# AdamQLMeng/PPNet

Hardware: AMD Instinct MI355X
Metric: edage_pp_map_path_instances_per_sec (higher is better)
Workload: dtype f64

## Files before the change

### include/ppnet_hip.h

```cpp
#ifndef PPNET_HIP_H
#define PPNET_HIP_H

#include <stdint.h>

#ifdef __cplusplus
extern "C" {
#endif

#define PPN_OK             0
#define PPN_E_INVALID     -1
#define PPN_E_HIP         -2
#define PPN_E_UNSUPPORTED -3

#define PPN_SEGS            10
#define PPN_POLY             5
#define PPN_PATH_POINTS   1000
#define PPN_BOUNDARY_POINTS 1100
#define PPN_DRAWS_PER_SEG 1002
#define PPN_DRAWS_PER_PATH (1 + PPN_SEGS * PPN_DRAWS_PER_SEG)
#define PPN_MAX_HULL        64
#define PPN_MAX_ISLES       16
#define PPN_MAX_POCKET      64
#define PPN_POCKET_TRY_CAP 256
#define PPN_PLACE_TRY_CAP 4096
// ... 285 lines not shown
                      void* stream);
#define PPN_AUG_FLIP            1u
#define PPN_AUG_BRIGHTNESS      2u
#define PPN_AUG_CONTRAST        4u
#define PPN_AUG_CONTRAST_LAST   8u
#define PPN_AUG_SATURATION     16u
#define PPN_AUG_HUE            32u
#define PPN_AUG_PARAM_WORDS     8
int ppn_augment_params(uint64_t seed, uint64_t first_instance, int B, double flip_ratio, double brightness_delta, double contrast_lo,
                       double contrast_hi, double saturation_lo, double saturation_hi, int hue_delta,
                       uint32_t* params , void* stream);
int ppn_augment_codes(const uint8_t* grid , const uint8_t* label_in ,
                      const uint32_t* params , void* img_out ,
                      uint8_t* label_out , int B, int H, int W, int Ho, int Wo,
                      const float* mean3, const float* std3, int seg_pad_val, int dtype , void* stream);
int ppn_augment_rgb(const uint8_t* rgb , const uint8_t* label_in ,
                    const uint32_t* params , void* img_out ,
                    uint8_t* label_out , int B, int H, int W, int Ho, int Wo,
                    const float* mean3, const float* std3, int seg_pad_val, int dtype , void* stream);
int ppn_seg_labels_2class(const void* logits, uint8_t* labels, int32_t B, int32_t h, int32_t w, int32_t Ho, int32_t Wo,
                          int32_t dtype, void* stream);
int ppn_bias_act_nhwc(void* x, const void* bias, int64_t n, int32_t C, float negative_slope, int32_t dtype, void* stream);

int ppn_conv3x3_c1_nhwc(const void* x, const float* w, const float* bias, void* y, int32_t B, int32_t H, int32_t W,
                        int32_t Cout, float negative_slope, int32_t dtype, void* stream);
int ppn_conv3x3_to1_nhwc(const void* x, const float* w, float bias, void* y, int32_t B, int32_t H, int32_t W, int32_t Cin,
                         int32_t dtype, void* stream);

int ppn_conv3x3_mfma_bf16(const void* x, const void* w, const float* bias, void* y, int32_t B, int32_t H, int32_t W, int32_t Cin,
                          int32_t Cout, int32_t stride, int32_t relu, void* stream);
int32_t ppn_conv3x3_relu_classify2_slots(int32_t Cout);
int ppn_conv3x3_relu_classify2_bf16(const void* x, const void* w, const float* bias, const float* w2, float* logits, float* partial, int32_t B,
                                    int32_t H, int32_t W, int32_t Cin, int32_t Cout, void* stream);
int ppn_gennet_conv_s2_bf16(const void* x, const void* w, const float* bias, void* y, int32_t B, int32_t H, int32_t W, float negative_slope,
                            int32_t transposed, void* stream);
int ppn_gennet_dec_final_bf16(const void* x, const void* w, const float* bias, float negative_slope, const float* w_final, float bias_final, void* y,
                              int32_t B, int32_t H, int32_t W, void* stream);
int ppn_gennet_first_enc_bf16(const void* x1, const void* w1, const float* b1, const void* wk2, const float* bias2, void* y, int32_t B, int32_t H, int32_t W,
                              float slope1, float slope2, void* stream);
#define PPN_GENNET_BLOCK_PARAMS 7224
int ppn_gennet_trunk_bf16(const void* x, void* y, const float* params, int32_t B, int32_t N, int32_t n_blocks, void* stream);
int ppn_assemble_paths(const double* wp, const int32_t* wp_n, const uint8_t* ok, const double* init, const double* end, double rate, int32_t n,
                       int32_t max_wp, double* full, int32_t* counts, void* stream);
int ppn_plan_collision(const double* waypoints, const int32_t* counts, const void* obstacles, int32_t obstacles_f64, const int32_t* n_obstacles,
                       int32_t B, int32_t M, int32_t S, float clearance, float bound, uint8_t* collision, void* stream);
int ppn_heatmap_u8(const void* y, uint8_t* out, int32_t B, int32_t n, int32_t dtype, void* stream);
int ppn_tokenizer_conv1_codes_bf16(const uint8_t* grid, const void* lut, void* out, int32_t B, int32_t H, int32_t W, void* stream);
int ppn_tokenizer_codes_bf16(const uint8_t* grid, const void* lut, const void* w2p, const float* vec, void* tokens, int32_t B, int32_t H, int32_t W,
                             float eps, void* stream);
int ppn_nat128_ln_qkv_bf16(const void* s, const float* offset, const void* ln_w, const void* ln_b, const void* w, const void* bias, void* qkv,
                           int64_t tokens, float eps, void* stream);
int ppn_nat128_ln_mlp_bf16(void* s, const float* offset, const void* ln_w, const void* ln_b, const void* w1, const void* b1, const void* w2,
                           int64_t tokens, float eps, void* stream);
int ppn_nat128_ln_mlp_add_bf16(void* s, const float* offset, const void* ln_w, const void* ln_b, const void* w1, const void* b1, const void* w2,
                               const float* final_add, int64_t tokens, float eps, void* stream);
int ppn_nat128_proj_add_bf16(void* s, const void* a, const void* w, int64_t tokens, void* stream);

int ppn_gemm_bf16(const void* a, const void* w, const float* bias, void* c, int64_t M, int32_t N, int32_t K, int32_t epilogue,
                  int32_t persistent_blocks, void* stream);

int32_t ppn_nat_gemm_partials(int32_t C);

int ppn_nat_gemm_bf16(const void* a, const void* w, const float* bias, const float* colsum, const float* stats_in, int32_t partials_in,
                      float* stats_out, void* c, int64_t M, int32_t N, int32_t K, int32_t mode, float eps, void* stream);

int32_t ppn_nat_mlp_supported(int64_t M, int32_t C, int32_t HID);
// ... 17 lines not shown
```

### ppnet_amd/_lib.py

```python
import ctypes as C
import os

_HERE = os.path.dirname(os.path.abspath(__file__))
LIB_PATH = os.environ.get("PPNET_HIP_LIB") or os.path.join(_HERE, "libppnet_hip.so")

PPN_OK = 0
PPN_E_UNSUPPORTED = -3
SEGS = 10
PATH_POINTS = 1000
BOUNDARY_POINTS = 1100
DRAWS_PER_SEG = 1002
DRAWS_PER_PATH = 1 + SEGS * DRAWS_PER_SEG
MAX_HULL = 64
MAX_ISLES = 16
MAX_POCKET = 64
POCKET_TRY_CAP = 256
PLACE_TRY_CAP = 4096
MAX_WAYPOINTS = 2048
GRID_OBST, GRID_FREE, GRID_MARK = 0, 255, 128
FLAG_POCKET_CAP, FLAG_PLACE_CAP, FLAG_EMPTY_ISLE, FLAG_HULL_CAP, FLAG_ISLE_CAP, FLAG_POCKET_FULL = 1, 2, 4, 8, 16, 32
FLAG_CORRIDOR_PASS = 64
FLAG_POCKET_DRAWS = 128

_p = C.c_void_p
# ... 9 lines not shown

class MapsStruct(C.Structure):
    _fields_ = [(n, _p) for n in (
        "grid", "angle", "translation", "attempts", "segpoint", "pathpoint", "accept", "obstacles",
        "n_obstacles", "flags", "records")]


class TtaAug(C.Structure):
    _fields_ = [("logit", _p), ("h", C.c_int32), ("w", C.c_int32), ("hm", C.c_int32), ("wm", C.c_int32), ("flip", C.c_int32)]


ABI_VERSION = 111

EXPORTS = ("ppn_version", "ppn_error_string", "ppn_last_hip_error", "ppn_polyfit_table", "ppn_edage_paths",
           "ppn_edage_paths_ex", "ppn_edage_paths_ex2", "ppn_edage_maps", "ppn_edage_maps_place", "ppn_edage_maps_raster",
           "ppn_label_masks", "ppn_boundary_check", "ppn_boundary_check_ex",
           "ppn_obstacle_filter", "ppn_paint_markers", "ppn_disc_raster", "ppn_collision_segments", "ppn_collision_segments_bound",
           "ppn_extract_paths", "ppn_resize_bilinear_u8", "ppn_philox_doubles", "ppn_na2d_fwd", "ppn_na2d_fwd_padded", "ppn_na2d_fwd_vpad", "ppn_swin_wmsa_fwd", "ppn_swin_wmsa_bwd", "ppn_swin_wmsa_bwd_workspace", "ppn_mhsa_fwd", "ppn_mhsa_bwd", "ppn_mhsa_bwd_workspace", "ppn_na2d_bwd", "ppn_na2d_bwd_workspace", "ppn_na2d_bwd_vpad", "ppn_na2d_bwd_vpad_workspace", "ppn_residual_layernorm", "ppn_residual_layernorm_padded", "ppn_layernorm_offset", "ppn_upsample2x_nhwc", "ppn_resize_concat4_nhwc", "ppn_resize_concat_nhwc", "ppn_adaptive_pools_nhwc", "ppn_upsample2x_add_nhwc", "ppn_upsample2x_nhwc_bias", "ppn_upsample2x_concat_nhwc", "ppn_bias_act_nhwc", "ppn_seg_labels_2class", "ppn_grid_to_image", "ppn_conv3x3_c1_nhwc", "ppn_conv3x3_to1_nhwc",
           "ppn_conv3x3_mfma_bf16", "ppn_conv3x3_relu_classify2_bf16", "ppn_conv3x3_relu_classify2_slots", "ppn_gemm_bf16", "ppn_nat_gemm_bf16", "ppn_nat_gemm_partials", "ppn_row_stats_bf16", "ppn_nat_mlp_supported", "ppn_nat_mlp_pack_bf16", "ppn_nat_mlp_bf16", "ppn_gennet_conv_s2_bf16", "ppn_gennet_trunk_bf16",
           "ppn_assemble_paths", "ppn_plan_collision", "ppn_gennet_first_enc_bf16", "ppn_gennet_dec_final_bf16", "ppn_heatmap_u8", "ppn_tokenizer_conv1_codes_bf16", "ppn_tokenizer_codes_bf16", "ppn_nat128_ln_qkv_bf16", "ppn_nat128_ln_mlp_bf16", "ppn_nat128_ln_mlp_add_bf16", "ppn_nat128_proj_add_bf16",
           "ppn_resize_ce_workspace", "ppn_resize_ce_fwd", "ppn_resize_ce_bwd", "ppn_seg_eval",
           "ppn_augment_params", "ppn_augment_codes", "ppn_augment_rgb",
           "ppn_ohem_ce_workspace", "ppn_ohem_ce_fwd", "ppn_ohem_ce_bwd",
           "ppn_resize_dice_workspace", "ppn_resize_dice_fwd", "ppn_resize_dice_bwd",
           "ppn_upsample2x_nhwc_bwd", "ppn_upsample2x_concat_nhwc_bwd", "ppn_resize_concat_nhwc_bwd",
           "ppn_residual_layernorm_train_fwd", "ppn_residual_layernorm_bwd_workspace", "ppn_residual_layernorm_bwd",
           "ppn_patch_merge_ln_fwd", "ppn_patch_merge_ln_bwd_workspace", "ppn_patch_merge_ln_bwd", "ppn_patch_merge_ln_rows",
           "ppn_patch_merge_ln_max_blocks", "ppn_seg_tta",
           "ppn_gennet_stem_train_workspace", "ppn_gennet_stem_train_fwd", "ppn_gennet_stem_train_bwd", "ppn_gennet_stem_train_tile",
           "ppn_gennet_stem_train_max_blocks",
           "ppn_gennet_tail_train_workspace", "ppn_gennet_tail_train_fwd", "ppn_gennet_tail_train_bwd", "ppn_gennet_tail_train_tile",
           "ppn_gennet_tail_train_max_blocks",
           "ppn_gennet_s2_tile", "ppn_gennet_s2_max_blocks", "ppn_gennet_s2_wgrad_workspace", "ppn_gennet_s2_down", "ppn_gennet_s2_up",
           "ppn_gennet_s2_wgrad")


def _load():
    if not os.path.exists(LIB_PATH):
        raise ImportError(
            f"{LIB_PATH} is missing: the HIP extension is the only implementation of this package "
            f"(no CPU fallback). Build it with `python -c 'import __graft_entry__ as g; g.build()'` "
            f"or `make -C ppnet_amd/csrc`.")
    lib = C.CDLL(LIB_PATH)
    lib.ppn_version.restype = C.c_int
    if lib.ppn_version() != ABI_VERSION:
        raise ImportError(
            f"{LIB_PATH} reports ABI version {lib.ppn_version()}, these bindings are written against {ABI_VERSION} "
            f"(include/ppnet_hip.h: PPN_ABI_VERSION): argument lists differ, rebuild with `make -C ppnet_amd/csrc`.")
    lib.ppn_error_string.restype = C.c_char_p
    lib.ppn_error_string.argtypes = [C.c_int]
    lib.ppn_last_hip_error.restype = C.c_int
    lib.ppn_polyfit_table.argtypes = [_p]
    lib.ppn_edage_paths.argtypes = [C.c_int32, C.c_uint64, C.c_int32, C.c_double, C.c_double, C.c_uint64,
                                    _p, _p, C.c_int32, C.POINTER(PathsStruct), _p]
    lib.ppn_edage_paths_ex.argtypes = [C.c_int32, C.c_uint64, C.c_int32, C.c_double, C.c_double, C.c_uint64,
                                       _p, _p, C.c_int32, _p, C.POINTER(PathsStruct), _p]
    lib.ppn_edage_paths_ex2.argtypes = [C.c_int32, C.c_uint64, C.c_int32, C.c_double, C.c_double, C.c_uint64,
                                        _p, _p, C.c_int32, _p, _p, C.POINTER(PathsStruct), _p]
    lib.ppn_boundary_check_ex.argtypes = [_p, C.c_int32, _p, _p, C.c_int32, C.c_int32, _p, _p, _p]
    lib.ppn_obstacle_filter.argtypes = [_p, _p, C.c_int32, C.c_int32, C.c_int32, C.c_double, C.c_double, C.c_double,
                                        _p, _p, _p, _p]
    lib.ppn_paint_markers.argtypes = [_p, C.c_int32, C.c_int32, _p, _p, _p]
    lib.ppn_edage_maps.argtypes = [C.POINTER(PathsStruct), C.c_int32, C.c_int32, C.c_uint64, C.c_int32,
                                   C.c_double, C.c_double, C.c_int32, C.c_double, C.c_uint64, _p, _p,
                                   C.POINTER(MapsStruct), _p]
    lib.ppn_edage_maps_place.argtypes = lib.ppn_edage_maps.argtypes
    lib.ppn_edage_maps_raster.argtypes = [C.POINTER(PathsStruct), C.c_int32, C.c_int32, C.c_int32, C.c_int32,
# ... 48 lines not shown
    lib.ppn_patch_merge_ln_fwd.argtypes = [_p] * 5 + [C.c_int] * 4 + [C.c_float, C.c_int, _p]
    lib.ppn_patch_merge_ln_bwd_workspace.argtypes = [C.c_int] * 4
    lib.ppn_patch_merge_ln_bwd_workspace.restype = C.c_int64
    lib.ppn_patch_merge_ln_bwd.argtypes = [_p] * 8 + [C.c_int] * 5 + [_p]
    lib.ppn_patch_merge_ln_rows.argtypes = [C.c_int]
    lib.ppn_patch_merge_ln_max_blocks.argtypes = []
    lib.ppn_gennet_stem_train_workspace.argtypes = [C.c_int] * 4
    lib.ppn_gennet_stem_train_workspace.restype = C.c_int64
    lib.ppn_gennet_stem_train_fwd.argtypes = [_p] * 9 + [C.c_int] * 4 + [C.c_float, C.c_float, C.c_int, _p]
    lib.ppn_gennet_stem_train_bwd.argtypes = [_p] * 12 + [C.c_int] * 4 + [C.c_float, C.c_int, _p]
    lib.ppn_gennet_stem_train_tile.argtypes = []
    lib.ppn_gennet_stem_train_max_blocks.argtypes = []
    lib.ppn_gennet_tail_train_workspace.argtypes = [C.c_int] * 4
    lib.ppn_gennet_tail_train_workspace.restype = C.c_int64
    lib.ppn_gennet_tail_train_fwd.argtypes = [_p] * 8 + [C.c_int] * 4 + [C.c_float, C.c_float, C.c_int, _p]
    lib.ppn_gennet_tail_train_bwd.argtypes = [_p] * 12 + [C.c_int] * 4 + [C.c_float, C.c_int, _p]
    lib.ppn_gennet_tail_train_tile.argtypes = []
    lib.ppn_gennet_tail_train_max_blocks.argtypes = []
    lib.ppn_gennet_s2_tile.argtypes = []
    lib.ppn_gennet_s2_max_blocks.argtypes = []
    lib.ppn_gennet_s2_wgrad_workspace.argtypes = [C.c_int] * 3
    lib.ppn_gennet_s2_wgrad_workspace.restype = C.c_int64
    lib.ppn_gennet_s2_down.argtypes = [_p] * 4 + [C.c_int] * 5 + [_p]
    lib.ppn_gennet_s2_up.argtypes = [_p] * 4 + [C.c_int] * 5 + [_p]
    lib.ppn_gennet_s2_wgrad.argtypes = [_p] * 6 + [C.c_int] * 5 + [_p]
    lib.ppn_grid_to_image.argtypes = [_p, _p, C.c_int64, C.POINTER(C.c_float), C.POINTER(C.c_float), C.c_int32, _p]
    lib.ppn_seg_labels_2class.argtypes = [_p, _p, C.c_int32, C.c_int32, C.c_int32, C.c_int32, C.c_int32, C.c_int32, _p]
    lib.ppn_bias_act_nhwc.argtypes = [_p, _p, C.c_int64, C.c_int32, C.c_float, C.c_int32, _p]
    lib.ppn_conv3x3_c1_nhwc.argtypes = [_p, _p, _p, _p, C.c_int32, C.c_int32, C.c_int32, C.c_int32, C.c_float, C.c_int32, _p]
    lib.ppn_conv3x3_to1_nhwc.argtypes = [_p, _p, C.c_float, _p, C.c_int32, C.c_int32, C.c_int32, C.c_int32, C.c_int32, _p]
    lib.ppn_conv3x3_mfma_bf16.argtypes = [_p, _p, _p, _p, C.c_int32, C.c_int32, C.c_int32, C.c_int32, C.c_int32, C.c_int32, C.c_int32, _p]
    lib.ppn_conv3x3_relu_classify2_bf16.argtypes = [_p, _p, _p, _p, _p, _p, C.c_int32, C.c_int32, C.c_int32, C.c_int32, C.c_int32, _p]
    lib.ppn_conv3x3_relu_classify2_slots.argtypes = [C.c_int32]
    lib.ppn_gennet_conv_s2_bf16.argtypes = [_p, _p, _p, _p, C.c_int32, C.c_int32, C.c_int32, C.c_float, C.c_int32, _p]
    lib.ppn_gennet_trunk_bf16.argtypes = [_p, _p, _p, C.c_int32, C.c_int32, C.c_int32, _p]
    lib.ppn_assemble_paths.argtypes = [_p, _p, _p, _p, _p, C.c_double, C.c_int32, C.c_int32, _p, _p, _p]
    lib.ppn_plan_collision.argtypes = [_p, _p, _p, C.c_int32, _p, C.c_int32, C.c_int32, C.c_int32, C.c_float, C.c_float, _p, _p]
    lib.ppn_gennet_first_enc_bf16.argtypes = [_p, _p, _p, _p, _p, _p, C.c_int32, C.c_int32, C.c_int32, C.c_float, C.c_float, _p]
    lib.ppn_gennet_dec_final_bf16.argtypes = [_p, _p, _p, C.c_float, _p, C.c_float, _p, C.c_int32, C.c_int32, C.c_int32, _p]
    lib.ppn_heatmap_u8.argtypes = [_p, _p, C.c_int32, C.c_int32, C.c_int32, _p]
    lib.ppn_tokenizer_conv1_codes_bf16.argtypes = [_p, _p, _p, C.c_int32, C.c_int32, C.c_int32, _p]
    lib.ppn_tokenizer_codes_bf16.argtypes = [_p, _p, _p, _p, _p, C.c_int32, C.c_int32, C.c_int32, C.c_float, _p]
    lib.ppn_nat128_ln_qkv_bf16.argtypes = [_p, _p, _p, _p, _p, _p, _p, C.c_int64, C.c_float, _p]
    lib.ppn_nat128_ln_mlp_bf16.argtypes = [_p, _p, _p, _p, _p, _p, _p, C.c_int64, C.c_float, _p]
    lib.ppn_nat128_ln_mlp_add_bf16.argtypes = [_p, _p, _p, _p, _p, _p, _p, _p, C.c_int64, C.c_float, _p]
    lib.ppn_nat128_proj_add_bf16.argtypes = [_p, _p, _p, C.c_int64, _p]
    lib.ppn_gemm_bf16.argtypes = [_p, _p, _p, _p, C.c_int64, C.c_int32, C.c_int32, C.c_int32, C.c_int32, _p]
    lib.ppn_nat_gemm_bf16.argtypes = [_p, _p, _p, _p, _p, C.c_int32, _p, _p, C.c_int64, C.c_int32, C.c_int32, C.c_int32, C.c_float, _p]
    lib.ppn_row_stats_bf16.argtypes = [_p, C.c_int64, C.c_int32, _p, _p]
    lib.ppn_nat_gemm_partials.argtypes = [C.c_int32]
    lib.ppn_nat_mlp_supported.argtypes = [C.c_int64, C.c_int32, C.c_int32]
    lib.ppn_nat_mlp_pack_bf16.argtypes = [_p, _p, _p, C.c_int32, C.c_int32, _p]
    lib.ppn_nat_mlp_bf16.argtypes = [_p, _p, _p, _p, _p, C.c_int64, C.c_int32, C.c_int32, C.c_float, _p]
    lib.ppn_resize_ce_workspace.argtypes = [C.c_int] * 3
    lib.ppn_resize_ce_workspace.restype = C.c_int64
    lib.ppn_resize_ce_fwd.argtypes = [_p, _p, _p, _p, _p, _p, C.c_int64] + [C.c_int] * 9 + [_p]
    lib.ppn_resize_ce_bwd.argtypes = [_p, _p, _p, _p, _p] + [C.c_int] * 9 + [_p]
    lib.ppn_seg_eval.argtypes = [_p, _p, _p, _p] + [C.c_int] * 9 + [_p]
    lib.ppn_seg_tta.argtypes = [C.POINTER(TtaAug), C.c_int, _p, _p] + [C.c_int] * 5 + [_p]
    lib.ppn_ohem_ce_workspace.argtypes = [C.c_int] * 3
    lib.ppn_ohem_ce_workspace.restype = C.c_int64
    lib.ppn_ohem_ce_fwd.argtypes = [_p] * 10 + [C.c_int64] + [C.c_int] * 8 + [C.c_float] + [C.c_int] * 3 + [_p]
    lib.ppn_ohem_ce_bwd.argtypes = [_p] * 8 + [C.c_int] * 10 + [_p]
    lib.ppn_resize_dice_workspace.argtypes = [C.c_int] * 4
    lib.ppn_resize_dice_workspace.restype = C.c_int64
    lib.ppn_resize_dice_fwd.argtypes = [_p] * 8 + [C.c_int] * 7 + [C.c_float] + [C.c_int] * 2 + [_p]
# ... 32 lines not shown
```

### ppnet_amd/csrc/capi.hip

```cpp
#include <hip/hip_runtime.h>
#include <math.h>
#include <mutex>
#include <stdlib.h>
#include <string.h>
#include <vector>

#include <cstdlib>
#include "ppn_kernels.h"

namespace {

thread_local int g_last_hip = 0;

inline int hip_fail(hipError_t e) {
    g_last_hip = (int)e;
    return PPN_E_HIP;
}
#define PPN_HIP(call) do { hipError_t e_ = (call); if (e_ != hipSuccess) return hip_fail(e_); } while (0)

inline bool bad_R(int R) { return R < 32 || R > 512 || (R % 32) != 0; }

void build_polyfit_table(double* out) {
    const int N = PPN_PATH_POINTS, M = 5;
    std::vector<long double> q((size_t)M * N);
// ... 1086 lines not shown
                         void* stream) {
    if (!x || !w || !y || B <= 0 || H <= 0 || W <= 0 || Cin <= 0 || Cin > 32 || (Cin % 8) != 0 || (dtype != 0 && dtype != 1))
        return PPN_E_INVALID;
    const int e = ppn::conv3x3_to1_launch(x, w, bias, y, B, H, W, Cin, dtype, (hipStream_t)stream);
    if (e != 0) return hip_fail((hipError_t)e);
    return PPN_OK;
}

int ppn_conv3x3_mfma_bf16(const void* x, const void* w, const float* bias, void* y, int32_t B, int32_t H, int32_t W, int32_t Cin,
                          int32_t Cout, int32_t stride, int32_t relu, void* stream) {
    if (!x || !w || !bias || !y || B <= 0 || H <= 0 || W <= 0 || Cin <= 0 || (Cin % 64) != 0 || Cout <= 0 || (Cout % 8) != 0 ||
        (stride != 1 && stride != 2))
        return PPN_E_INVALID;
    if ((long long)B * H * W * Cin * 2 >= (1LL << 32) || (long long)Cout * 9 * Cin * 2 >= (1LL << 32) || (long long)B * H * W >= (1LL << 31))
        return PPN_E_UNSUPPORTED;
    const int e = ppn::conv3x3_mfma_launch(x, w, bias, y, B, H, W, Cin, Cout, stride, relu, nullptr, nullptr, nullptr, (hipStream_t)stream);
    if (e != 0) return hip_fail((hipError_t)e);
    return PPN_OK;
}

int32_t ppn_conv3x3_relu_classify2_slots(int32_t Cout) { return Cout > 0 ? (Cout > 256 ? (Cout + 255) / 256 : 0) : -1; }

int ppn_conv3x3_relu_classify2_bf16(const void* x, const void* w, const float* bias, const float* w2, float* logits, float* partial, int32_t B,
                                    int32_t H, int32_t W, int32_t Cin, int32_t Cout, void* stream) {
    if (!x || !w || !bias || !w2 || !logits || (!partial && Cout > 256) || B <= 0 || H <= 0 || W <= 0 || Cin <= 0 || (Cin % 64) != 0 || Cout <= 0 || (Cout % 8) != 0)
        return PPN_E_INVALID;
    if ((long long)B * H * W * Cin * 2 >= (1LL << 32) || (long long)Cout * 9 * Cin * 2 >= (1LL << 32) || (long long)B * H * W >= (1LL << 31))
        return PPN_E_UNSUPPORTED;
    const int e = ppn::conv3x3_mfma_launch(x, w, bias, nullptr, B, H, W, Cin, Cout, 1, 1, w2, logits, partial, (hipStream_t)stream);
    if (e != 0) return hip_fail((hipError_t)e);
    return PPN_OK;
}

int ppn_gennet_conv_s2_bf16(const void* x, const void* w, const float* bias, void* y, int32_t B, int32_t H, int32_t W, float negative_slope,
                            int32_t transposed, void* stream) {
    if (!x || !w || !bias || !y || B <= 0 || H <= 0 || W <= 0 || (!transposed && ((H | W) & 1))) return PPN_E_INVALID;
    if ((long long)B * H * W * 4 >= (1LL << 31)) return PPN_E_UNSUPPORTED;
    const int e = transposed ? ppn::gennet_dec_conv_launch(x, w, bias, y, B, H, W, negative_slope, (hipStream_t)stream)
                             : ppn::gennet_enc_conv_launch(x, w, bias, y, B, H, W, negative_slope, (hipStream_t)stream);
    if (e != 0) return hip_fail((hipError_t)e);
    return PPN_OK;
}

int ppn_gennet_first_enc_bf16(const void* x1, const void* w1, const float* b1, const void* wk2, const float* bias2, void* y, int32_t B, int32_t H, int32_t W,
                              float slope1, float slope2, void* stream) {
    if (!x1 || !w1 || !b1 || !wk2 || !bias2 || !y || B <= 0 || H <= 0 || W <= 0 || ((H | W) & 1)) return PPN_E_INVALID;
    const int e = ppn::gennet_first_enc_launch(x1, w1, b1, wk2, bias2, y, B, H, W, slope1, slope2, (hipStream_t)stream);
    if (e != 0) return hip_fail((hipError_t)e);
    return PPN_OK;
}

int ppn_gennet_dec_final_bf16(const void* x, const void* w, const float* bias, float negative_slope, const float* w_final, float bias_final, void* y,
                              int32_t B, int32_t H, int32_t W, void* stream) {
    if (!x || !w || !bias || !w_final || !y || B <= 0 || H <= 0 || W <= 0) return PPN_E_INVALID;
    if ((long long)B * H * W * 4 * 24 >= (1LL << 32)) return PPN_E_UNSUPPORTED;
    const int e = ppn::gennet_dec_final_launch(x, w, bias, negative_slope, w_final, bias_final, y, B, H, W, (hipStream_t)stream);
    if (e != 0) return hip_fail((hipError_t)e);
    return PPN_OK;
}

int ppn_gennet_trunk_bf16(const void* x, void* y, const float* params, int32_t B, int32_t N, int32_t n_blocks, void* stream) {
    if (!x || !y || !params || B <= 0 || N <= 0 || N > 1024 || (N % 8) != 0 || n_blocks <= 0) return PPN_E_INVALID;
    const int e = ppn::gennet_trunk_launch(x, y, params, B, N, n_blocks, (hipStream_t)stream);
    if (e != 0) return hip_fail((hipError_t)e);
    return PPN_OK;
}
// ... 163 lines not shown
```

### ppnet_amd/csrc/ppn_kernels.h

```cpp
#pragma once
#include <hip/hip_runtime.h>
#include <stdint.h>
#include <atomic>
#include "../../include/ppnet_hip.h"

#ifndef PPN_PATHS_THREADS
#define PPN_PATHS_THREADS 256
#endif

namespace ppn {

constexpr int PPN_MAX_DEVICES = 64;
inline int current_device() {
    int d = 0;
    return (hipGetDevice(&d) == hipSuccess && d >= 0 && d < PPN_MAX_DEVICES) ? d : -1;
}
struct DeviceOnce { std::atomic<int> done[PPN_MAX_DEVICES]; };
struct DeviceBuffer { std::atomic<void*> p[PPN_MAX_DEVICES]; };
inline int dynamic_lds_once(DeviceOnce& o, const void* fn, int bytes) {
    const int d = current_device();
    if (d < 0) return (int)hipErrorInvalidDevice;
    if (o.done[d].load(std::memory_order_acquire)) return 0;
    const hipError_t e = hipFuncSetAttribute(fn, hipFuncAttributeMaxDynamicSharedMemorySize, bytes);
    if (e != hipSuccess) return (int)e;
// ... 116 lines not shown
int gennet_tail_tile();
int gennet_tail_max_blocks();
long long gennet_tail_train_workspace_bytes(long long n, int C);
int gennet_tail_train_fwd_launch(const void* y, const float* gamma, const float* beta, const float* wf, const float* bf, void* out, float* stats,
                                 void* workspace, int B, int H, int W, int C, float eps, float slope, int dtype, hipStream_t stream);
int gennet_tail_train_bwd_launch(const void* dout, const void* y, const float* gamma, const float* beta, const float* wf, const float* stats,
                                 void* workspace, void* dy, float* dgamma, float* dbeta, float* dwf, float* dbf, int B, int H, int W, int C,
                                 float slope, int dtype, hipStream_t stream);

int gennet_s2_tile();
int gennet_s2_max_blocks();
long long gennet_s2_wgrad_workspace_bytes(long long ns);
int gennet_s2_down_launch(const void* big, const float* w, const float* bias, void* small, int B, int H, int W, int C, int dtype, hipStream_t stream);
int gennet_s2_up_launch(const void* small, const float* w, const float* bias, void* big, int B, int H, int W, int C, int dtype, hipStream_t stream);
int gennet_s2_wgrad_launch(const void* small, const void* big, void* workspace, float* dw, float* sum_small, float* sum_big, int B, int H, int W,
                           int C, int dtype, hipStream_t stream);

int resize_concat_launch(const void* const* x, const int* hw, const int* ch, int n, void* out, int B, int dtype, hipStream_t stream);
int adaptive_pools_launch(const void* x, void* const* y, const int* scales, int n, int B, int H, int W, int C, int dtype, hipStream_t stream);
int upsample2x_launch(const void* x, const void* bias, const void* add, void* y, int B, int H, int W, int C, int relu, int dtype, hipStream_t stream);
int upsample2x_concat_launch(const void* const* x, const int* ch, int n, void* y, int B, int H, int W, int dtype, hipStream_t stream);
int upsample2x_bwd_launch(const void* dy, const void* x, void* dx, int B, int H, int W, int C, int dtype, hipStream_t stream);
int upsample2x_concat_bwd_launch(const void* dout, void* const* dx, const int* ch, int n, int B, int H, int W, int dtype, hipStream_t stream);
int resize_concat_bwd_launch(const void* dout, void* const* dx, const int* hw, const int* ch, int n, int B, int dtype, hipStream_t stream);
int conv3x3_c1_launch(const void* x, const float* w, const float* bias, void* y, int B, int H, int W, int Cout, float slope, int dtype,
                      hipStream_t stream);
int conv3x3_to1_launch(const void* x, const float* w, float bias, void* y, int B, int H, int W, int Cin, int dtype, hipStream_t stream);
int seg_labels_launch(const void* lo, uint8_t* labels, int B, int h, int w, int Ho, int Wo, int dtype, hipStream_t stream);
int grid_image_launch(const uint8_t* grid, void* img, long long n, const float* mean, const float* stdv, int dtype, hipStream_t stream);
int bias_act_launch(void* x, const void* bias, long long n, int C, float slope, int dtype, hipStream_t stream);

int conv3x3_mfma_launch(const void* x, const void* w, const float* bias, void* y, int B, int H, int W, int Cin, int Cout, int stride,
                        int relu, const float* w2, float* logits, float* partial, hipStream_t stream);
int gennet_enc_conv_launch(const void* x, const void* wk, const float* bias, void* y, int B, int H, int W, float slope, hipStream_t stream);
int gennet_dec_conv_launch(const void* x, const void* wt, const float* bias, void* y, int B, int H, int W, float slope, hipStream_t stream);
int assemble_paths_launch(const double* wp, const int32_t* wp_n, const uint8_t* ok, const double* init, const double* end, double rate, int n, int max_wp,
                          double* full, int32_t* counts, hipStream_t stream);
int plan_collision_launch(const double* full, const int32_t* counts, const void* obstacles, int obs_f64, const int32_t* n_obs, int B, int M, int S,
                          float clearance, float bound, uint8_t* collision, hipStream_t stream);
int mhsa_launch(const void* qkv, void* out, int B, int N, int heads, float scale, int dtype, hipStream_t stream);
long long mhsa_bwd_workspace_floats(int B, int N, int heads);
int mhsa_bwd_launch(const void* qkv, const void* out, const void* dout, void* dqkv, float* workspace, int B, int N, int heads, float scale, int dtype,
                    hipStream_t stream);
int mhsa_d8_block_rows();
int mhsa_d8_block_threads();
int mhsa_d8_launch(const void* qkv, void* out, int B, int N, int heads, float scale, int dtype, hipStream_t stream);
int mhsa_d8_bwd_launch(const void* qkv, const void* out, const void* dout, void* dqkv, float* workspace, int B, int N, int heads, float scale,
                       int dtype, hipStream_t stream);
int swin_wmsa_launch(const void* qkv, const void* pad_kv, const float* rpb, void* out, int B, int H, int W, int heads, int shift, float scale,
                     int dtype, hipStream_t stream);
long long swin_wmsa_bwd_workspace_floats(int heads);
int swin_wmsa_bwd_launch(const void* qkv, const void* pad_kv, const float* rpb, const void* dout, void* dqkv, float* dpad_kv, float* drpb,
                         float* workspace, int B, int H, int W, int heads, int shift, float scale, int dtype, hipStream_t stream);
int resize_ce_fwd_pixels();
int resize_ce_threads();
int resize_ce_bwd_lanes(int h, int w, int H, int W);
long long resize_ce_workspace_floats(int B, int H, int W);
int resize_ce_fwd_launch(const void* logit, const void* label, float* lse, float* loss, int64_t* correct, float* workspace, int B, int C, int h,
                         int w, int H, int W, int ignore_index, int logit_dtype, int label_dtype, hipStream_t stream);
int resize_ce_bwd_launch(const void* logit, const void* label, const float* lse, const float* grad_out, void* dlogit, int B, int C, int h, int w,
                         int H, int W, int ignore_index, int logit_dtype, int label_dtype, hipStream_t stream);
int seg_eval_pixels();
int seg_eval_threads();
int seg_eval_max_groups();
int seg_eval_max_classes();
int seg_eval_launch(const void* logit, const void* label, uint8_t* pred, int64_t* areas, int B, int C, int h, int w, int H, int W, int ignore_index,
// ... 66 lines not shown
```

### ppnet_amd/fused.py

```python
import ctypes
import os

import torch
import torch.nn.functional as F
from torch.autograd.function import once_differentiable

from . import _lib as L

_DT = {torch.float32: 0, torch.bfloat16: 1}


def _p(t):
    return ctypes.c_void_p(t.data_ptr()) if t is not None else ctypes.c_void_p(None)


class WeightCache:
    __slots__ = ("key", "value", "__weakref__")
    _all = None

    def __init__(self):
        self.key = self.value = None
        if WeightCache._all is None:
            import weakref
            WeightCache._all = weakref.WeakSet()
# ... 651 lines not shown
    if not x.is_contiguous():
        x = x.contiguous()
    B, H, W, Cin = x.shape
    Cout = w_k.shape[0]
    Ho, Wo = (H - 1) // stride + 1, (W - 1) // stride + 1
    assert w_k.dtype == torch.bfloat16 and w_k.is_contiguous() and w_k.shape == (Cout, 3, 3, Cin)
    assert bias32.dtype == torch.float32 and bias32.is_contiguous() and bias32.numel() == Cout
    y = torch.empty(B, Ho, Wo, Cout, dtype=x.dtype, device=x.device)
    with torch.cuda.device(x.device):
        rc = L.lib.ppn_conv3x3_mfma_bf16(_p(x), _p(w_k), _p(bias32), _p(y), B, H, W, Cin, Cout, stride, 1 if relu else 0,
                                         ctypes.c_void_p(torch.cuda.current_stream(x.device).cuda_stream))
    L.check(rc, "ppn_conv3x3_mfma_bf16")
    return y.permute(0, 3, 1, 2)


def conv3x3_relu_classify2(x_nchw_cl, w_k, bias32, w2_32, b2_32):
    if not x_nchw_cl.is_cuda or x_nchw_cl.dtype != torch.bfloat16:
        raise RuntimeError("ppnet_amd.fused.conv3x3_relu_classify2: bfloat16 GPU tensors only")
    x = x_nchw_cl.permute(0, 2, 3, 1)
    if not x.is_contiguous():
        x = x.contiguous()
    B, H, W, Cin = x.shape
    Cout = w_k.shape[0]
    logits = b2_32.to(torch.float32).repeat(B * H * W).view(B, H, W, 2).contiguous()
    slots = L.lib.ppn_conv3x3_relu_classify2_slots(Cout)
    partial = torch.empty(slots, B * H * W, 2, dtype=torch.float32, device=x.device) if slots > 0 else None
    with torch.cuda.device(x.device):
        rc = L.lib.ppn_conv3x3_relu_classify2_bf16(_p(x), _p(w_k), _p(bias32), _p(w2_32), _p(logits), _p(partial), B, H, W, Cin, Cout,
                                                   ctypes.c_void_p(torch.cuda.current_stream(x.device).cuda_stream))
    L.check(rc, "ppn_conv3x3_relu_classify2_bf16")
    return logits.permute(0, 3, 1, 2)


def gemm_bf16(a, w, bias32, epilogue="bias", out=None, persistent_blocks=0):
    epi = {"bias": 0, "bias_gelu": 1, "accum": 2, "bias_relu": 3}[epilogue]
    M, K = a.shape
    N = w.shape[0]
    assert a.is_cuda and a.dtype == torch.bfloat16 and w.dtype == torch.bfloat16 and a.is_contiguous() and w.is_contiguous()
    if out is None:
        assert epi != 2
        out = torch.empty(M, N, dtype=a.dtype, device=a.device)
    assert out.is_contiguous() and out.shape == (M, N)
    with torch.cuda.device(a.device):
        rc = L.lib.ppn_gemm_bf16(_p(a), _p(w), _p(bias32), _p(out), M, N, K, epi, persistent_blocks,
                                 ctypes.c_void_p(torch.cuda.current_stream(a.device).cuda_stream))
    L.check(rc, "ppn_gemm_bf16")
    return out


def nat_gemm(a, w, bias32, mode, out, colsum=None, stats_in=None, stats_out=None, eps=1e-5):
    md = {"ln": 0, "ln_gelu": 1, "acc": 2}[mode]
    M, K = a.shape
    N = w.shape[0]
    assert a.is_cuda and a.dtype == w.dtype == out.dtype == torch.bfloat16 and a.is_contiguous() and w.is_contiguous() and out.is_contiguous()
    assert w.shape == (N, K) and out.shape == (M, N) and bias32.dtype == torch.float32 and bias32.numel() == N and bias32.is_contiguous()
    P = 0
    if md != 2:
        assert colsum.dtype == torch.float32 and colsum.numel() == N and colsum.is_contiguous()
        assert stats_in.dtype == torch.float32 and stats_in.is_contiguous() and stats_in.dim() == 3 and stats_in.shape[1:] == (M, 2)
        P = stats_in.shape[0]
    else:
        assert stats_out.dtype == torch.float32 and stats_out.is_contiguous() and stats_out.shape == (nat_partials(N), M, 2)
    with torch.cuda.device(a.device):
        rc = L.lib.ppn_nat_gemm_bf16(_p(a), _p(w), _p(bias32), _p(colsum), _p(stats_in), P, _p(stats_out), _p(out), M, N, K, md, float(eps),
                                     ctypes.c_void_p(torch.cuda.current_stream(a.device).cuda_stream))
    L.check(rc, "ppn_nat_gemm_bf16")
# ... 954 lines not shown
```

### ppnet_amd/heads.py

```python
import os

import torch
import torch.nn as nn
import torch.nn.functional as F

from . import fused
from .dense import mfma_weights, use_mfma_conv


class _BatchNorm2d(nn.BatchNorm2d):

    def forward(self, x):
        if self.weight is not None and x.dtype != self.weight.dtype:
            x = x.to(self.weight.dtype)
        return super().forward(x)


class _ConvModule(nn.Sequential):

    def __init__(self, cin, cout, k, dilation=1):
        super().__init__()
        self.add_module("conv", nn.Conv2d(cin, cout, k, 1, ((k - 1) // 2) * dilation, dilation, bias=False))
        self.add_module("bn", _BatchNorm2d(cout))
        self.add_module("activate", nn.ReLU(inplace=True))
# ... 72 lines not shown


def _loss_specs(loss_decode, num_classes):
    if loss_decode is None:
        entries = [{}]
    elif isinstance(loss_decode, dict):
        entries = [loss_decode]
    elif isinstance(loss_decode, (list, tuple)) and len(loss_decode) > 0 and all(isinstance(d, dict) for d in loss_decode):
        entries = list(loss_decode)
    else:
        raise TypeError(f"loss_decode must be a dict or a non-empty sequence of dicts, got {loss_decode!r}")
    single = _single_ce(loss_decode)
    specs = []
    for d in entries:
        typ = d.get("type", _CE)
        if typ not in (_CE, _DICE):
            raise NotImplementedError(f"loss type {typ!r}: CrossEntropyLoss and DiceLoss only (LovaszLoss, FocalLoss and the rest are not built)")
        if not single:
            if d.get("use_sigmoid", False):
                raise NotImplementedError(f"{typ}(use_sigmoid=True): sigmoid / binary cross-entropy is not built")
            if d.get("reduction", "mean") != "mean":
                raise NotImplementedError(f"{typ}(reduction={d['reduction']!r}): 'mean' only")
        spec = dict(type=typ, loss_name=str(d.get("loss_name", "loss_ce" if typ == _CE else "loss_dice")),
                    loss_weight=float(d.get("loss_weight", 1.0)), class_weight=_class_weight_entry(d.get("class_weight"), num_classes))
        if typ == _DICE:
            ignore = d.get("ignore_index", 255)
            spec.update(smooth=float(d.get("smooth", 1)), exponent=d.get("exponent", 2), ignore_index=-1 if ignore is None else int(ignore))
            if not spec["smooth"] >= 0.0:
                raise ValueError(f"DiceLoss(smooth={d.get('smooth')!r}): not negative")
        specs.append(spec)
    return tuple(specs)


class SETRUPHead(nn.Module):
    def __init__(self, in_channels=1024, channels=512, num_classes=2, num_convs=1, up_scale=4, kernel_size=3,
                 in_index=-1, dropout_ratio=0.1, align_corners=False, norm_layer=None, norm_cfg=None, sampler=None, loss_decode=None,
                 **kwargs):
        super().__init__()
        assert kernel_size in (1, 3)
        self.in_index, self.align_corners = in_index, align_corners
        self.sampler, self.class_weight = _loss_options(sampler, loss_decode, num_classes)
        self.loss_specs, self.loss_single_ce = _loss_specs(loss_decode, num_classes), _single_ce(loss_decode)
        self.norm = nn.LayerNorm(in_channels, eps=1e-6)
        self.up_convs = nn.ModuleList()
        cin = in_channels
        for _ in range(num_convs):
            self.up_convs.append(nn.Sequential(_ConvModule(cin, channels, kernel_size), _Upsample(up_scale, align_corners)))
            cin = channels
        self.conv_seg = nn.Conv2d(channels, num_classes, 1)
        self.dropout = nn.Dropout2d(dropout_ratio) if dropout_ratio > 0 else nn.Identity()

    def forward(self, inputs, lowres=False):
        x = inputs[self.in_index]
        x = fused.layer_norm_any_width(x.permute(0, 2, 3, 1), self.norm).permute(0, 3, 1, 2)
        prepared = all(isinstance(up[0].bn, nn.Identity) and up[0].conv.bias is not None for up in self.up_convs)
        if prepared and all(use_mfma_conv(x, up[0].conv) for up in self.up_convs) and self.conv_seg.out_channels == 2:
            return self._forward_mfma(x, lowres)
        for up in self.up_convs[:-1]:
            cm = up[0]
            if isinstance(cm.bn, nn.Identity) and cm.conv.bias is not None:
                c = cm.conv
                x = up[1](F.conv2d(x, c.weight, None, c.stride, c.padding), relu=True, bias=c.bias)
            else:
                x = up[1](cm.bn(cm.conv(x)), relu=True)
        conv, up = self.up_convs[-1][0], self.up_convs[-1][1]
        if isinstance(conv.bn, nn.Identity) and conv.conv.bias is not None and x.is_cuda:
            c = conv.conv
            y = fused.bias_act_(F.conv2d(x, c.weight, None, c.stride, c.padding).contiguous(memory_format=torch.channels_last), c.bias, 0.0)
        else:
            y = conv(x)
        if self.training:
            return self.conv_seg(self.dropout(up(y)))
        lo = self.conv_seg(y).contiguous()
        return lo if lowres else up(lo)

    _mfma = None

    def _forward_mfma(self, x, lowres):
        if self._mfma is None:
            self._mfma = fused.WeightCache()
        cs = self.conv_seg
        src = [t for up in self.up_convs for t in (up[0].conv.weight, up[0].conv.bias)] + [cs.weight, cs.bias]
        packs = self._mfma.get(src, lambda: [mfma_weights(up[0].conv) for up in self.up_convs] + [_seg_pack(cs)])
        n = len(self.up_convs) - 1

        def run(feats):
            x, = feats
            for i, up in enumerate(self.up_convs[:-1]):
                x = up[1](fused.conv3x3_mfma(x, packs[i][0], packs[i][1], stride=1, relu=True))
            lo = fused.conv3x3_relu_classify2(x, *packs[n], *packs[-1]).to(x.dtype).contiguous()
            return lo if lowres else self.up_convs[-1][1](lo)
        last_in = self.up_convs[-1][0].conv.in_channels * x.shape[-2] * x.shape[-1] * 4 ** n * 2
        return _in_equal_slices([x], max(1, (2 ** 32 - 1) // last_in), run)


class UPerHead(nn.Module):

    def __init__(self, in_channels=(128, 256, 512, 1024), channels=64, num_classes=2, pool_scales=(1, 2, 3, 6),
                 in_index=(0, 1, 2, 3), dropout_ratio=0.1, align_corners=False, norm_cfg=None, sampler=None, loss_decode=None, **kwargs):
        super().__init__()
        self.in_index, self.align_corners = tuple(in_index), align_corners
        self.sampler, self.class_weight = _loss_options(sampler, loss_decode, num_classes)
        self.loss_specs, self.loss_single_ce = _loss_specs(loss_decode, num_classes), _single_ce(loss_decode)
        self.psp_modules = nn.ModuleList(
            nn.Sequential(nn.AdaptiveAvgPool2d(ps), _ConvModule(in_channels[-1], channels, 1)) for ps in pool_scales)
        self.bottleneck = _ConvModule(in_channels[-1] + len(pool_scales) * channels, channels, 3)
        self.lateral_convs = nn.ModuleList(_ConvModule(c, channels, 1) for c in in_channels[:-1])
        self.fpn_convs = nn.ModuleList(_ConvModule(channels, channels, 3) for _ in in_channels[:-1])
        self.fpn_bottleneck = _ConvModule(len(in_channels) * channels, channels, 3)
        self.conv_seg = nn.Conv2d(channels, num_classes, 1)

    def _resize(self, x, size):
        if (x.is_cuda and not self.align_corners and tuple(size) == (2 * x.shape[2], 2 * x.shape[3]) and x.shape[1] % 8 == 0
                and x.dtype in (torch.float32, torch.bfloat16) and not (fused.library_upsample() and fused.recording(x))):
            return fused.upsample2x_nhwc(x)
        return F.interpolate(x, size=size, mode="bilinear", align_corners=self.align_corners)

    _packs = None

    def _prepared_mfma(self, x):
        cms = [m for m in self.modules() if isinstance(m, _ConvModule)]
        return (x.is_cuda and x.dtype == torch.bfloat16 and not self.training and all(isinstance(c.bn, nn.Identity) and c.conv.bias is not None for c in cms)
                and self.conv_seg.out_channels == 2 and not fused.recording(x, self.conv_seg.weight) and not os.environ.get("PPNET_LIBRARY_CONV"))
# ... 385 lines not shown
```

Before: 57.64 million.

## Compute 3x3 conv after 2x bilinear upsample via low-res tap GEMM and fused tap-sum

Swaps the order of bilinear 2x upsampling and the following 3x3 conv in the SETR-UP head. A GEMM first produces per-tap outputs (9*Cout channels) at low resolution. A new HIP kernel then combines those taps with the bilinear weights, adds bias and applies ReLU, and in the last stage can also fuse the 2-class classifier. This avoids materializing the upsampled activation and running the conv at 4x the pixels, but it writes a 9*Cout-wide intermediate, and the classify path reduces across lanes with shuffles.

```diff
diff --git a/include/ppnet_hip.h b/include/ppnet_hip.h
--- a/include/ppnet_hip.h
+++ b/include/ppnet_hip.h
@@ -341,6 +341,9 @@
 int32_t ppn_conv3x3_relu_classify2_slots(int32_t Cout);
 int ppn_conv3x3_relu_classify2_bf16(const void* x, const void* w, const float* bias, const float* w2, float* logits, float* partial, int32_t B,
                                     int32_t H, int32_t W, int32_t Cin, int32_t Cout, void* stream);
+int ppn_tapsum_up2_relu_bf16(const void* T, const float* bias, void* y, int32_t B, int32_t H, int32_t W, int32_t Cout, void* stream);
+int ppn_tapsum_up2_relu_classify2_bf16(const void* T, const float* bias, const float* w2, const float* b2, float* logits, int32_t B, int32_t H,
+                                       int32_t W, int32_t Cout, void* stream);
 int ppn_gennet_conv_s2_bf16(const void* x, const void* w, const float* bias, void* y, int32_t B, int32_t H, int32_t W, float negative_slope,
                             int32_t transposed, void* stream);
 int ppn_gennet_dec_final_bf16(const void* x, const void* w, const float* bias, float negative_slope, const float* w_final, float bias_final, void* y,
diff --git a/ppnet_amd/_lib.py b/ppnet_amd/_lib.py
--- a/ppnet_amd/_lib.py
+++ b/ppnet_amd/_lib.py
@@ -65,7 +65,7 @@
            "ppn_gennet_tail_train_workspace", "ppn_gennet_tail_train_fwd", "ppn_gennet_tail_train_bwd", "ppn_gennet_tail_train_tile",
            "ppn_gennet_tail_train_max_blocks",
            "ppn_gennet_s2_tile", "ppn_gennet_s2_max_blocks", "ppn_gennet_s2_wgrad_workspace", "ppn_gennet_s2_down", "ppn_gennet_s2_up",
-           "ppn_gennet_s2_wgrad")
+           "ppn_gennet_s2_wgrad", "ppn_tapsum_up2_relu_bf16", "ppn_tapsum_up2_relu_classify2_bf16")
 
 
 def _load():
@@ -180,6 +180,8 @@
     lib.ppn_conv3x3_mfma_bf16.argtypes = [_p, _p, _p, _p, C.c_int32, C.c_int32, C.c_int32, C.c_int32, C.c_int32, C.c_int32, C.c_int32, _p]
     lib.ppn_conv3x3_relu_classify2_bf16.argtypes = [_p, _p, _p, _p, _p, _p, C.c_int32, C.c_int32, C.c_int32, C.c_int32, C.c_int32, _p]
     lib.ppn_conv3x3_relu_classify2_slots.argtypes = [C.c_int32]
+    lib.ppn_tapsum_up2_relu_bf16.argtypes = [_p, _p, _p, C.c_int32, C.c_int32, C.c_int32, C.c_int32, _p]
+    lib.ppn_tapsum_up2_relu_classify2_bf16.argtypes = [_p, _p, _p, _p, _p, C.c_int32, C.c_int32, C.c_int32, C.c_int32, _p]
     lib.ppn_gennet_conv_s2_bf16.argtypes = [_p, _p, _p, _p, C.c_int32, C.c_int32, C.c_int32, C.c_float, C.c_int32, _p]
     lib.ppn_gennet_trunk_bf16.argtypes = [_p, _p, _p, C.c_int32, C.c_int32, C.c_int32, _p]
     lib.ppn_assemble_paths.argtypes = [_p, _p, _p, _p, _p, C.c_double, C.c_int32, C.c_int32, _p, _p, _p]
diff --git a/ppnet_amd/csrc/capi.hip b/ppnet_amd/csrc/capi.hip
--- a/ppnet_amd/csrc/capi.hip
+++ b/ppnet_amd/csrc/capi.hip
@@ -1142,6 +1142,31 @@
     return PPN_OK;
 }
 
+static int tapsum_up2_check(const void* T, const float* bias, const void* out, size_t out_align, int32_t B, int32_t H, int32_t W, int32_t Cout) {
+    if (!T || !bias || !out || B <= 0 || H <= 0 || W <= 0 || Cout <= 0 || (Cout % 8) != 0 || ((uintptr_t)T & 15) != 0 ||
+        ((uintptr_t)out & (out_align - 1)) != 0)
+        return PPN_E_INVALID;
+    return ppn::tapsum_up2_supported(B, H, W) ? PPN_OK : PPN_E_UNSUPPORTED;
+}
+
+int ppn_tapsum_up2_relu_bf16(const void* T, const float* bias, void* y, int32_t B, int32_t H, int32_t W, int32_t Cout, void* stream) {
+    const int c = tapsum_up2_check(T, bias, y, 16, B, H, W, Cout);
+    if (c != PPN_OK) return c;
+    const int e = ppn::tapsum_up2_launch(T, bias, nullptr, nullptr, y, nullptr, B, H, W, Cout, (hipStream_t)stream);
+    if (e != 0) return hip_fail((hipError_t)e);
+    return PPN_OK;
+}
+
+int ppn_tapsum_up2_relu_classify2_bf16(const void* T, const float* bias, const float* w2, const float* b2, float* logits, int32_t B, int32_t H,
+                                       int32_t W, int32_t Cout, void* stream) {
+    if (!w2 || !b2) return PPN_E_INVALID;
+    const int c = tapsum_up2_check(T, bias, logits, 8, B, H, W, Cout);
+    if (c != PPN_OK) return c;
+    const int e = ppn::tapsum_up2_launch(T, bias, w2, b2, nullptr, logits, B, H, W, Cout, (hipStream_t)stream);
+    if (e != 0) return hip_fail((hipError_t)e);
+    return PPN_OK;
+}
+
 int ppn_gennet_conv_s2_bf16(const void* x, const void* w, const float* bias, void* y, int32_t B, int32_t H, int32_t W, float negative_slope,
                             int32_t transposed, void* stream) {
     if (!x || !w || !bias || !y || B <= 0 || H <= 0 || W <= 0 || (!transposed && ((H | W) & 1))) return PPN_E_INVALID;
diff --git a/ppnet_amd/csrc/ppn_kernels.h b/ppnet_amd/csrc/ppn_kernels.h
--- a/ppnet_amd/csrc/ppn_kernels.h
+++ b/ppnet_amd/csrc/ppn_kernels.h
@@ -172,6 +172,9 @@
 
 int conv3x3_mfma_launch(const void* x, const void* w, const float* bias, void* y, int B, int H, int W, int Cin, int Cout, int stride,
                         int relu, const float* w2, float* logits, float* partial, hipStream_t stream);
+bool tapsum_up2_supported(long long B, long long H, long long W);
+int tapsum_up2_launch(const void* T, const float* bias, const float* w2, const float* b2, void* y, float* logits, int B, int H, int W, int Cout,
+                      hipStream_t stream);
 int gennet_enc_conv_launch(const void* x, const void* wk, const float* bias, void* y, int B, int H, int W, float slope, hipStream_t stream);
 int gennet_dec_conv_launch(const void* x, const void* wt, const float* bias, void* y, int B, int H, int W, float slope, hipStream_t stream);
 int assemble_paths_launch(const double* wp, const int32_t* wp_n, const uint8_t* ok, const double* init, const double* end, double rate, int n, int max_wp,
diff --git a/ppnet_amd/csrc/tap_upconv.hip b/ppnet_amd/csrc/tap_upconv.hip
--- /dev/null
+++ b/ppnet_amd/csrc/tap_upconv.hip
@@ -0,0 +1,188 @@
+#include <hip/hip_runtime.h>
+#include <stdint.h>
+#include "ppn_kernels.h"
+#include "resize_tap.h"
+
+namespace ppn {
+
+namespace {
+
+constexpr int TU_ROWS = 4;
+constexpr int TU_SEG = 32;
+
+struct AxisWeights { float a[4], b[4]; };
+
+__device__ __forceinline__ AxisWeights axis_weights(int i, int n) {
+    AxisWeights w;
+#pragma unroll
+    for (int p = 0; p < 4; ++p) {
+        const int P = 2 * i - 1 + p;
+        w.a[p] = w.b[p] = 0.f;
+        if (P >= 0 && P < 2 * n) {
+            const Tap t = bilinear_tap(P, n, 2 * n);
+            const int s = i - 1 + (p >> 1);
+            w.a[p] = tap_weight(t, s);
+            w.b[p] = tap_weight(t, s + 1);
+        }
+    }
+    return w;
+}
+
+__device__ __forceinline__ void load8(const uint16_t* p, float (&v)[8]) {
+    const uint4 u = *reinterpret_cast<const uint4*>(p);
+    v[0] = __uint_as_float(u.x << 16); v[1] = __uint_as_float(u.x & 0xffff0000u);
+    v[2] = __uint_as_float(u.y << 16); v[3] = __uint_as_float(u.y & 0xffff0000u);
+    v[4] = __uint_as_float(u.z << 16); v[5] = __uint_as_float(u.z & 0xffff0000u);
+    v[6] = __uint_as_float(u.w << 16); v[7] = __uint_as_float(u.w & 0xffff0000u);
+}
+
+__device__ __forceinline__ uint32_t bf16_bits(float v) {
+    const __bf16 h = (__bf16)v;
+    return (uint32_t)(*reinterpret_cast<const uint16_t*>(&h));
+}
+
+struct ColR { float r[3][2][8]; };
+
+__device__ __forceinline__ void column_r(const uint16_t* t0, const uint16_t* t1, const uint16_t* t2, size_t col_off, int Cout, const AxisWeights& wv,
+                                         ColR& out) {
+    const uint16_t* rows[3] = {t0 + col_off, t1 + col_off, t2 + col_off};
+#pragma unroll
+    for (int kx = 0; kx < 3; ++kx) {
+        float v[3][3][8];
+#pragma unroll
+        for (int s = 0; s < 3; ++s)
+#pragma unroll
+            for (int ky = 0; ky < 3; ++ky) load8(rows[s] + (size_t)(3 * ky + kx) * Cout, v[s][ky]);
+#pragma unroll
+        for (int y = 0; y < 2; ++y)
+#pragma unroll
+            for (int k = 0; k < 8; ++k) {
+                float acc = 0.f;
+#pragma unroll
+                for (int ky = 0; ky < 3; ++ky) {
+                    const int p = y + ky, s = p >> 1;
+                    acc = fmaf(wv.a[p], v[s][ky][k], acc);
+                    acc = fmaf(wv.b[p], v[s + 1][ky][k], acc);
+                }
+                out.r[kx][y][k] = acc;
+            }
+    }
+}
+
+}
+
+template <bool CLASSIFY>
+__global__ __launch_bounds__(64 * TU_ROWS) void tapsum_up2_kernel(const uint16_t* __restrict__ T, const float* __restrict__ bias,
+                                                                  const float* __restrict__ w2, const float* __restrict__ b2,
+                                                                  uint16_t* __restrict__ y, float* __restrict__ logits, int H, int W, int Cout,
+                                                                  int row_blocks, int segs) {
+    const int lane = threadIdx.x & 63, wave = threadIdx.x >> 6;
+    const int seg = (int)(blockIdx.x % (unsigned)segs);
+    const int rb = (int)((blockIdx.x / (unsigned)segs) % (unsigned)row_blocks);
+    const int b = (int)(blockIdx.x / ((unsigned)segs * (unsigned)row_blocks));
+    const int i = rb * TU_ROWS + wave;
+    if (i >= H) return;
+    const int j0 = seg * TU_SEG, j1 = min(j0 + TU_SEG, W);
+    const AxisWeights wv = axis_weights(i, H);
+    const size_t row_len = (size_t)W * 9 * Cout;
+    const uint16_t* img = T + (size_t)b * H * row_len;
+    const size_t cell = (size_t)9 * Cout;
+
+    for (int cbase = 0; cbase < Cout; cbase += 512) {
+        const bool live = cbase + lane * 8 < Cout;
+        const int c0 = live ? cbase + lane * 8 : 0;
+        const uint16_t* t0 = img + (size_t)max(i - 1, 0) * row_len + c0;
+        const uint16_t* t1 = img + (size_t)i * row_len + c0;
+        const uint16_t* t2 = img + (size_t)min(i + 1, H - 1) * row_len + c0;
+        float bv[8], wc[2][8];
+#pragma unroll
+        for (int k = 0; k < 8; ++k) bv[k] = bias[c0 + k];
+        if constexpr (CLASSIFY) {
+#pragma unroll
+            for (int k = 0; k < 8; ++k) { wc[0][k] = live ? w2[c0 + k] : 0.f; wc[1][k] = live ? w2[Cout + c0 + k] : 0.f; }
+        }
+        ColR rm, rc, rn;
+#pragma unroll
+        for (int kx = 0; kx < 3; ++kx)
+#pragma unroll
+            for (int yy = 0; yy < 2; ++yy)
+#pragma unroll
+                for (int k = 0; k < 8; ++k) rm.r[kx][yy][k] = rc.r[kx][yy][k] = 0.f;
+
+        for (int jj = j0 - 1; jj <= j1; ++jj) {
+            if (jj >= 0 && jj < W) {
+                column_r(t0, t1, t2, (size_t)jj * cell, Cout, wv, rn);
+            } else {
+#pragma unroll
+                for (int kx = 0; kx < 3; ++kx)
+#pragma unroll
+                    for (int yy = 0; yy < 2; ++yy)
+#pragma unroll
+                        for (int k = 0; k < 8; ++k) rn.r[kx][yy][k] = 0.f;
+            }
+            const int j = jj - 1;
+            if (j >= j0) {
+                const AxisWeights wh = axis_weights(j, W);
+#pragma unroll
+                for (int yy = 0; yy < 2; ++yy)
+#pragma unroll
+                    for (int xx = 0; xx < 2; ++xx) {
+                        float o[8];
+#pragma unroll
+                        for (int k = 0; k < 8; ++k) {
+                            float acc = 0.f;
+#pragma unroll
+                            for (int kx = 0; kx < 3; ++kx) {
+                                const int q = xx + kx;
+                                const float ra = q < 2 ? rm.r[kx][yy][k] : rc.r[kx][yy][k];
+                                const float rb2 = q < 2 ? rc.r[kx][yy][k] : rn.r[kx][yy][k];
+                                acc = fmaf(wh.a[q], ra, acc);
+                                acc = fmaf(wh.b[q], rb2, acc);
+                            }
+                            o[k] = fmaxf(bv[k] + acc, 0.f);
+                        }
+                        const size_t pix = ((size_t)b * 2 * H + (2 * i + yy)) * 2 * W + (2 * j + xx);
+                        if constexpr (CLASSIFY) {
+                            float l0 = 0.f, l1 = 0.f;
+#pragma unroll
+                            for (int k = 0; k < 8; ++k) { l0 = fmaf(wc[0][k], o[k], l0); l1 = fmaf(wc[1][k], o[k], l1); }
+#pragma unroll
+                            for (int s = 32; s > 0; s >>= 1) { l0 += __shfl_xor(l0, s, 64); l1 += __shfl_xor(l1, s, 64); }
+                            if (lane == 0) {
+                                float2* dst = reinterpret_cast<float2*>(logits) + pix;
+                                const float2 prev = cbase == 0 ? make_float2(b2[0], b2[1]) : *dst;
+                                *dst = make_float2(prev.x + l0, prev.y + l1);
+                            }
+                        } else {
+                            if (live)
+                                *reinterpret_cast<uint4*>(y + pix * Cout + c0) =
+                                    make_uint4(bf16_bits(o[0]) | (bf16_bits(o[1]) << 16), bf16_bits(o[2]) | (bf16_bits(o[3]) << 16),
+                                               bf16_bits(o[4]) | (bf16_bits(o[5]) << 16), bf16_bits(o[6]) | (bf16_bits(o[7]) << 16));
+                        }
+                    }
+            }
+            rm = rc;
+            rc = rn;
+        }
+    }
+}
+
+bool tapsum_up2_supported(long long B, long long H, long long W) {
+    const long long blocks = B * ((H + TU_ROWS - 1) / TU_ROWS) * ((W + TU_SEG - 1) / TU_SEG);
+    return B * H * W * 4 < (1LL << 31) && blocks < (1LL << 31);
+}
+
+int tapsum_up2_launch(const void* T, const float* bias, const float* w2, const float* b2, void* y, float* logits, int B, int H, int W, int Cout,
+                      hipStream_t stream) {
+    const int row_blocks = (H + TU_ROWS - 1) / TU_ROWS, segs = (W + TU_SEG - 1) / TU_SEG;
+    const dim3 grid((unsigned)((long long)B * row_blocks * segs)), block(64 * TU_ROWS);
+    if (logits)
+        hipLaunchKernelGGL(tapsum_up2_kernel<true>, grid, block, 0, stream, (const uint16_t*)T, bias, w2, b2, (uint16_t*)nullptr, logits, H, W, Cout,
+                           row_blocks, segs);
+    else
+        hipLaunchKernelGGL(tapsum_up2_kernel<false>, grid, block, 0, stream, (const uint16_t*)T, bias, (const float*)nullptr, (const float*)nullptr,
+                           (uint16_t*)y, (float*)nullptr, H, W, Cout, row_blocks, segs);
+    return (int)hipGetLastError();
+}
+
+}
diff --git a/ppnet_amd/fused.py b/ppnet_amd/fused.py
--- a/ppnet_amd/fused.py
+++ b/ppnet_amd/fused.py
@@ -707,6 +707,48 @@
     return logits.permute(0, 3, 1, 2)
 
 
+def tap_weights(weight):
+    Cout, Cin = weight.shape[:2]
+    return weight.detach().permute(2, 3, 0, 1).reshape(9 * Cout, Cin).contiguous()
+
+
+_ZERO_BIAS = {}
+
+
+def _zero_bias(n, device):
+    z = _ZERO_BIAS.get((n, device))
+    if z is None:
+        z = _ZERO_BIAS[(n, device)] = torch.zeros(n, dtype=torch.float32, device=device)
+    return z
+
+
+def tap_upconv(r_nchw_cl, w9, bias32, w2_32=None, b2_32=None):
+    if not r_nchw_cl.is_cuda or r_nchw_cl.dtype != torch.bfloat16:
+        raise RuntimeError("ppnet_amd.fused.tap_upconv: bfloat16 GPU tensors only")
+    r = r_nchw_cl.permute(0, 2, 3, 1)
+    if not r.is_contiguous():
+        r = r.contiguous()
+    B, H, W, Cin = r.shape
+    Cout = w9.shape[0] // 9
+    assert w9.dtype == torch.bfloat16 and w9.is_contiguous() and w9.shape == (9 * Cout, Cin)
+    assert bias32.dtype == torch.float32 and bias32.is_contiguous() and bias32.numel() == Cout
+    cus = torch.cuda.get_device_properties(r.device).multi_processor_count // 8 * 8
+    T = gemm_bf16(r.reshape(B * H * W, Cin), w9, _zero_bias(9 * Cout, r.device), "bias", persistent_blocks=cus)
+    stream = ctypes.c_void_p(torch.cuda.current_stream(r.device).cuda_stream)
+    with torch.cuda.device(r.device):
+        if w2_32 is None:
+            out = torch.empty(B, 2 * H, 2 * W, Cout, dtype=r.dtype, device=r.device)
+            rc = L.lib.ppn_tapsum_up2_relu_bf16(_p(T), _p(bias32), _p(out), B, H, W, Cout, stream)
+            name = "ppn_tapsum_up2_relu_bf16"
+        else:
+            assert w2_32.dtype == b2_32.dtype == torch.float32 and w2_32.is_contiguous() and w2_32.shape == (2, Cout) and b2_32.numel() == 2
+            out = torch.empty(B, 2 * H, 2 * W, 2, dtype=torch.float32, device=r.device)
+            rc = L.lib.ppn_tapsum_up2_relu_classify2_bf16(_p(T), _p(bias32), _p(w2_32), _p(b2_32.contiguous()), _p(out), B, H, W, Cout, stream)
+            name = "ppn_tapsum_up2_relu_classify2_bf16"
+    L.check(rc, name)
+    return out.permute(0, 3, 1, 2)
+
+
 def gemm_bf16(a, w, bias32, epilogue="bias", out=None, persistent_blocks=0):
     epi = {"bias": 0, "bias_gelu": 1, "accum": 2, "bias_relu": 3}[epilogue]
     M, K = a.shape
diff --git a/ppnet_amd/heads.py b/ppnet_amd/heads.py
--- a/ppnet_amd/heads.py
+++ b/ppnet_amd/heads.py
@@ -128,6 +128,10 @@
     return tuple(specs)
 
 
+TAP_UPCONV_MIN_TOKENS = {"store": 256, "classify": 16384}
+TAP_UPCONV_SLICE_BYTES = None
+
+
 class SETRUPHead(nn.Module):
     def __init__(self, in_channels=1024, channels=512, num_classes=2, num_convs=1, up_scale=4, kernel_size=3,
                  in_index=-1, dropout_ratio=0.1, align_corners=False, norm_layer=None, norm_cfg=None, sampler=None, loss_decode=None,
@@ -172,19 +176,43 @@
 
     _mfma = None
 
+    def _tap_stage(self, i, r):
+        up = self.up_convs[i - 1][1]
+        if up.scale_factor != 2.0 or up.align_corners or os.environ.get("PPNET_NO_TAP_UPCONV"):
+            return False
+        floor = TAP_UPCONV_MIN_TOKENS["classify" if i == len(self.up_convs) - 1 else "store"]
+        return floor is not None and i >= len(self.up_convs) - 2 and r.shape[0] * r.shape[2] * r.shape[3] >= floor
+
     def _forward_mfma(self, x, lowres):
         if self._mfma is None:
             self._mfma = fused.WeightCache()
         cs = self.conv_seg
+        n = len(self.up_convs) - 1
         src = [t for up in self.up_convs for t in (up[0].conv.weight, up[0].conv.bias)] + [cs.weight, cs.bias]
-        packs = self._mfma.get(src, lambda: [mfma_weights(up[0].conv) for up in self.up_convs] + [_seg_pack(cs)])
-        n = len(self.up_convs) - 1
+        packs = self._mfma.get(src, lambda: [mfma_weights(up[0].conv) for up in self.up_convs] + [_seg_pack(cs)]
+                               + [{i: fused.tap_weights(self.up_convs[i][0].conv.weight) for i in range(max(1, n - 1), n + 1)}])
+        seg, w9 = packs[n + 1], packs[n + 2]
+
+        def tap(i, r):
+            hw, cout = r.shape[2] * r.shape[3], w9[i].shape[0] // 9
+            bmax = min((2 ** 32 - 1) // (hw * r.shape[1] * 2), (2 ** 31 - 1) // (4 * hw))
+            if TAP_UPCONV_SLICE_BYTES:
+                bmax = min(bmax, TAP_UPCONV_SLICE_BYTES // (hw * 9 * cout * 2))
+            cls = seg if i == n else (None, None)
+            return _in_equal_slices([r], max(1, bmax), lambda f: fused.tap_upconv(f[0], w9[i], packs[i][1], *cls))
 
         def run(feats):
             x, = feats
-            for i, up in enumerate(self.up_convs[:-1]):
-                x = up[1](fused.conv3x3_mfma(x, packs[i][0], packs[i][1], stride=1, relu=True))
-            lo = fused.conv3x3_relu_classify2(x, *packs[n], *packs[-1]).to(x.dtype).contiguous()
+            r = None
+            for i, up in enumerate(self.up_convs):
+                if r is not None and self._tap_stage(i, r):
+                    r = tap(i, r)
+                    continue
+                if r is not None:
+                    x = self.up_convs[i - 1][1](r)
+                r = (fused.conv3x3_relu_classify2(x, *packs[n], *seg) if i == n
+                     else fused.conv3x3_mfma(x, packs[i][0], packs[i][1], stride=1, relu=True))
+            lo = r.to(x.dtype).contiguous()
             return lo if lowres else self.up_convs[-1][1](lo)
         last_in = self.up_convs[-1][0].conv.in_channels * x.shape[-2] * x.shape[-1] * 4 ** n * 2
         return _in_equal_slices([x], max(1, (2 ** 32 - 1) // last_in), run)
```

After: 55.24 million. 0.958x the previous value.
